# Borx25/CPU-Raytracing-experiments

Measured on AMD Instinct MI355X. Metric: Mray/s (primary+bounce), higher is better.
Workload: dtype f32; 1 GPU; cfg4: 4096x4096 px, S(100000) spheres + SAH BVH, MIS, Policy.max_bounces=9 (primary+8 bounces), 5 buckets, 64 accumulations/step; fixed image, tile rows split over the GPUs; image=4096x4096, spheres=100000, max_bounces=9, buckets=5, parallelism=single GPU, batches_in_flight=1, accumulations_per_batch=63, accumulations_per_batch_limit=63

## Files before the change

cpu-raytracing-experiments_amd/csrc/kernels.hpp:

```cpp
#pragma once
#include <hip/hip_runtime.h>
#include <stdint.h>
#include "device_math.hpp"

namespace mirt {

constexpr uint32_t kBlock = 256;
constexpr uint32_t kShadeBlock = 512;
constexpr uint32_t kTraceBlock = 1024;
constexpr uint32_t kLdsStack = 16;
constexpr uint32_t kLdsStackWide = 12;
constexpr uint32_t kLeafBit = 0x80000000u;
constexpr uint32_t kTileSize = 256;
constexpr uint32_t kTileRoot = 16;
constexpr uint32_t kStack = 64;
constexpr uint32_t kDestAccum = 0x80000000u;

struct SceneDev {
	const float4* recs;
	const float4* spheres;
	const int32_t* prim_mat;
	const float4* light_sphere;
	const float4* light_emit;
	const float4* mat_albedo;
// ... 578 lines not shown
		out.path[i] = path;
	}
}

template <int MODE, bool COUNT, class LoadRay, class StoreResult>
MIRT_DI void trace_queue(const SceneDev& sc, const TraceLds tl, const Queue& q, uint32_t n, uint32_t* work_next, FatList fat, uint32_t& c_nodes, uint32_t& c_spheres,
                         LoadRay load_ray, StoreResult store_result, const Collect col = Collect{ nullptr, 0.0f, 0u }) {
	if (n == 0) return;
	const bool all = bvh_all_in_lds(sc);
	if (sc.half_boxes && sc.wide) {
		if (!sc.stack16) trace_persistent<MODE, COUNT, false, true, false, true>(sc, tl, q, n, work_next, fat, c_nodes, c_spheres, load_ray, store_result, col);
		else if (all) trace_persistent<MODE, COUNT, true, true, true, true>(sc, tl, q, n, work_next, fat, c_nodes, c_spheres, load_ray, store_result, col);
		else trace_persistent<MODE, COUNT, false, true, true, true>(sc, tl, q, n, work_next, fat, c_nodes, c_spheres, load_ray, store_result, col);
	} else if (sc.half_boxes) {
		if (!sc.stack16) trace_persistent<MODE, COUNT, false, true, false, false>(sc, tl, q, n, work_next, fat, c_nodes, c_spheres, load_ray, store_result, col);
		else if (all) trace_persistent<MODE, COUNT, true, true, true, false>(sc, tl, q, n, work_next, fat, c_nodes, c_spheres, load_ray, store_result, col);
		else trace_persistent<MODE, COUNT, false, true, true, false>(sc, tl, q, n, work_next, fat, c_nodes, c_spheres, load_ray, store_result, col);
	} else {
		if (all) trace_persistent<MODE, COUNT, true, false, false, false>(sc, tl, q, n, work_next, fat, c_nodes, c_spheres, load_ray, store_result, col);
		else trace_persistent<MODE, COUNT, false, false, false, false>(sc, tl, q, n, work_next, fat, c_nodes, c_spheres, load_ray, store_result, col);
	}
}

MIRT_DI size_t accum_index(uint32_t acc_base, uint32_t buckets, uint32_t pix_bits, uint32_t path) {
	const uint32_t slot = path >> pix_bits;
	const uint32_t pix = path & ((1u << pix_bits) - 1u);
	const uint32_t bucket = (acc_base + slot + 1u) % buckets;
	return (static_cast<size_t>(pix >> 8) * buckets + bucket) * 3u * kTileSize + (pix & 255u);
}
MIRT_DI size_t accum_index(const FrameParams& fp, uint32_t path) { return accum_index(fp.idx_base, fp.idx_buckets, fp.pix_bits, path); }
MIRT_DI void accumulate_add(float* __restrict__ accum, size_t idx, float r, float g, float b) {
	accum[idx] += r; accum[idx + kTileSize] += g; accum[idx + 2 * kTileSize] += b;
}
constexpr uint32_t kDestFull = 0x40000000u;
constexpr uint32_t kDestSlot = 0x3fffffffu;
struct ShadowSink {
	float *rr, *rg, *rb;
	const float *px, *py, *pz;
	float* accum;
	uint32_t acc_base, buckets, pix_bits;
	uint32_t* occ;
};
MIRT_DI void shadow_origin(const ShadowBuf& sh, const ShadowSink& sink, uint32_t i, float& px, float& py, float& pz) {
	if (sink.occ) { px = sh.px[i]; py = sh.py[i]; pz = sh.pz[i]; return; }
	const uint32_t dw = sh.dest[i];
	if (dw & kDestAccum) { px = sh.px[i]; py = sh.py[i]; pz = sh.pz[i]; }
	else { const uint32_t d = dw & kDestSlot; px = sink.px[d]; py = sink.py[d]; pz = sink.pz[d]; }
}
MIRT_DI void shadow_finish(const ShadowBuf& sh, const ShadowSink& sink, uint32_t i, bool occluded, uint32_t& c_term) {
	if (sink.occ) { sink.occ[i] = occluded ? 1u : 0u; return; }
	const uint32_t dw = sh.dest[i];
	const uint32_t dest = dw & (kDestSlot | kDestAccum);
	if (dw & kDestAccum) c_term++;
	if (dw & kDestFull) {
		f3 R{ sh.rr[i], sh.rg[i], sh.rb[i] };
		const f3 E{ sh.er[i], sh.eg[i], sh.eb[i] };
		if (!occluded) { R.x += sh.sr[i]; R.y += sh.sg[i]; R.z += sh.sb[i]; }
		R.x += E.x; R.y += E.y; R.z += E.z;
		if (dest & kDestAccum) accumulate_add(sink.accum, accum_index(sink.acc_base, sink.buckets, sink.pix_bits, dest & ~kDestAccum), R.x, R.y, R.z);
		else { sink.rr[dest] = R.x; sink.rg[dest] = R.y; sink.rb[dest] = R.z; }
	} else if (!occluded) {
		const f3 S{ sh.sr[i], sh.sg[i], sh.sb[i] };
		if (dest & kDestAccum) accumulate_add(sink.accum, accum_index(sink.acc_base, sink.buckets, sink.pix_bits, dest & ~kDestAccum), S.x, S.y, S.z);
		else { sink.rr[dest] += S.x; sink.rg[dest] += S.y; sink.rb[dest] += S.z; }
	}
}

constexpr int kPrimaryNone = 0, kPrimaryAll = 1, kPrimaryList = 2;
MIRT_DI uint32_t primary_list_ray(const FrameParams& fp, const uint32_t* __restrict__ ov_pix, uint32_t n_ov, float inv_n_ov, uint32_t j) {
	uint32_t k;
	const uint32_t slot = udiv_f(j, n_ov, inv_n_ov, k);
	return slot * fp.n_pix + ov_pix[k];
}
template <bool COUNT, int PRIMARY>
__global__ __launch_bounds__(kTraceBlock, 8) void k_trace(SceneDev sc, FrameParams fp,
                                                       StreamBuf in, HitRec* __restrict__ hit_out,
                                                       Queue closest_queue, uint32_t* closest_work,
                                                       ShadowBuf sh, ShadowSink sink,
                                                       Queue shadow_queue, uint32_t* shadow_work, FatList fat_closest, FatList fat_shadow,
                                                       DevCounters* ctr) {
	extern __shared__ float4 lds[];
	const uint32_t n_ov = PRIMARY == kPrimaryList ? closest_queue.n[0] : 0u;
	const float inv_n_ov = 1.0f / static_cast<float>(n_ov ? n_ov : 1u);
	if (PRIMARY) closest_queue.n = nullptr;
	const uint32_t nc = PRIMARY == kPrimaryAll ? fp.n_pix * fp.batch_n : PRIMARY == kPrimaryList ? n_ov * fp.batch_n : queue_total(closest_queue), ns = PRIMARY ? 0u : queue_total(shadow_queue);
	if (nc + ns == 0) return;
	if (blockIdx.x == 0 && threadIdx.x == 0) {
		if (nc && PRIMARY != kPrimaryList) atomicAdd(&ctr->rays, static_cast<unsigned long long>(nc));
		if (ns) atomicAdd(&ctr->shadow_rays, static_cast<unsigned long long>(ns));
	}
	uint32_t c_nodes = 0, c_spheres = 0, s_nodes = 0, s_spheres = 0, c_term = 0;
	if (sc.use_bvh && sc.n_recs != 0) {
		if (static_cast<uint64_t>(blockIdx.x) * 64u >= static_cast<uint64_t>(nc) + ns) return;
		const TraceLds tl = stage_bvh(sc, lds);
		{
			auto load_ray = [&](uint32_t i, float& px, float& py, float& pz, float& dx, float& dy, float& dz, float& tf) {
// ... 231 lines not shown
			}
			lane_on = pix < fp.n_pix;
			my_slot = slot_it * fp.n_pix + pix;
			if (lane_on) {
				uint32_t rng = hash_2d(fp.acc_base + slot_it + 1u, pix_seed);
				const float s0 = rand_unit_float(rng);
				const float s1 = rand_unit_float(rng);
				my_D = camera_ray_dir(fp.cam, pix_x, pix_y, s0, s1);
				my_path = (slot_it << fp.pix_bits) | pix;
				{ const HitRec h = hit_in[my_slot]; my_prim = h.prim; my_tfar = h.tfar; }
			}
			if (++slot_it == slot_end) unit += gridDim.x;
		} else {
			lane_on = base + threadIdx.x < n;
			const uint32_t nb = base + gridDim.x * kShadeBlock;
			next_slot = (nb + threadIdx.x < n) ? queue_slot(qin, nb, nb + threadIdx.x) : 0u;
			next_prim = hit_in[next_slot].prim;
			base = nb;
		}
		{
			if (lane_on) {
				const uint32_t i = my_slot;
				const int32_t prim = my_prim;
				if (prim < 0) {
					f3 R{0.0f, 0.0f, 0.0f};
					float thr_x = 1.0f;
					uint32_t mpath = my_path; f3 md = my_D;
					if (!FIRST) { R = { in.rr[i], in.rg[i], in.rb[i] }; thr_x = in.tr[i]; mpath = in.path[i]; }
					if (sc.has_ambient) {
						if (!FIRST) md = { in.dx[i], in.dy[i], in.dz[i] };
						const f3 sky = sky_eval(sc, md.x, md.y, md.z);
						R.x += thr_x * sky.x; R.y += thr_x * sky.y; R.z += thr_x * sky.z;
					}
					accumulate_add(accum, accum_index(fp, mpath), R.x + 0.0f, R.y + 0.0f, R.z + 0.0f);
					c_term++;
				} else if (last_bounce) {
					c_drop++;
				} else is_hit = true;
			}
		}
		const uint32_t n_hits = FIRST ? 0u : block_compact(is_hit, my_slot, compact_scratch, hit_list);

		bool survive = false, has_shadow = false, terminated = false, has_E = false;
		uint32_t path = 0;
		f3 P{0, 0, 0}, ndir{0, 0, 0}, L{0, 0, 0}, srad{0, 0, 0}, E{0, 0, 0};
		f3 R{0.0f, 0.0f, 0.0f}, thr{1.0f, 1.0f, 1.0f};
		float light_distance = 0.0f;
		if (FIRST ? is_hit : threadIdx.x < n_hits) {
			const uint32_t i = FIRST ? my_slot : hit_list[threadIdx.x];
			f3 D = my_D;
			path = my_path;
			if (!FIRST) { path = in.path[i]; D = { in.dx[i], in.dy[i], in.dz[i] }; }
			float pdf_in = 0.0f;
			if (!FIRST) {
				R = { in.rr[i], in.rg[i], in.rb[i] };
				thr = { in.tr[i], in.tg[i], in.tb[i] };
				pdf_in = MIRT_INV_PI * max_sel(0.0f, D.z);
			}
			const HitRec hrec = FIRST ? HitRec{ my_tfar, my_prim } : hit_in[i];
			const int32_t prim = hrec.prim;
			{
				const float depth = hrec.tfar;
				const float4 hs = sc.spheres[prim];
				const int32_t mat = sc.prim_mat[prim];
				const f3 O = FIRST ? f3{ fp.cam.pos[0], fp.cam.pos[1], fp.cam.pos[2] } : f3{ in.px[i], in.py[i], in.pz[i] };
				const f3 hit{ O.x + D.x * depth, O.y + D.y * depth, O.z + D.z * depth };
				f3 N = normalize3(f3{ hit.x - hs.x, hit.y - hs.y, hit.z - hs.z });
				if (dot3(N, D) >= 0.0f) N = f3{ -N.x, -N.y, -N.z };
				const quat T = tangent_space(N);
				const f3 Vl = to_local(T, f3{ -D.x, -D.y, -D.z });
// ... 42 lines not shown
					} while (false);
				}
				has_E = is_emissive;
				if (is_emissive) {
					if (fp.mis && bounce > 0) {
						const float radius2 = hs.w;
						const float center_dist2 = depth * (depth + Vl.z * (2.0f * __builtin_sqrtf(radius2))) + radius2;
						const float weight = powerHeuristic(pdf_in, light_selection_pdf * spherePdf(radius2, center_dist2));
						E = { (thr.x * weight) * em.x, (thr.y * weight) * em.y, (thr.z * weight) * em.z };
					} else {
						E = { em.x, em.y, em.z };
					}
				}
				{
					uint32_t rng = hash_2d(acc, seed + bounce * 2u + 1u);
					const float b0 = rand_unit_float(rng);
					const float b1 = rand_unit_float(rng);
					f3 sd = hemisphere(b0, b1);
					thr = { thr.x * alb.x, thr.y * alb.y, thr.z * alb.z };
					const float q = 1.0f - max_sel(thr.x, max_sel(thr.y, thr.z));
					if (rand_unit_float(rng) < q) {
						terminated = true;
					} else {
						const float inv = 1.0f / max_sel(MIRT_FLT_EPSILON, 1.0f - q);
						thr = { thr.x * inv, thr.y * inv, thr.z * inv };
						ndir = to_world(T, sd);
						survive = true;
					}
				}
			}
		}
		uint32_t slot, sslot;
		block_append2(survive, has_shadow, next_queue, shadow_queue, iteration % kSegs, append_scratch, parity, slot, sslot);
		const bool direct = fp.idx_base != 0xffffffffu;
		const bool full = has_shadow & (has_E | (terminated & direct));
		if (survive) {
			out.px[slot] = P.x; out.py[slot] = P.y; out.pz[slot] = P.z;
			out.dx[slot] = ndir.x; out.dy[slot] = ndir.y; out.dz[slot] = ndir.z;
			out.tr[slot] = thr.x; out.tg[slot] = thr.y; out.tb[slot] = thr.z;
			out.path[slot] = path;
		}
		if (has_shadow) {
			if (!survive) { sh.px[sslot] = P.x; sh.py[sslot] = P.y; sh.pz[sslot] = P.z; }
			sh.dx[sslot] = L.x; sh.dy[sslot] = L.y; sh.dz[sslot] = L.z;
			sh.tfar[sslot] = light_distance;
			sh.sr[sslot] = srad.x; sh.sg[sslot] = srad.y; sh.sb[sslot] = srad.z;
			if (full) {
				sh.rr[sslot] = R.x; sh.rg[sslot] = R.y; sh.rb[sslot] = R.z;
				sh.er[sslot] = E.x; sh.eg[sslot] = E.y; sh.eb[sslot] = E.z;
			}
			sh.dest[sslot] = (survive ? slot : (kDestAccum | path)) | (full ? kDestFull : 0u);
		}
		if ((survive | terminated) & !full) {
			const f3 Rf{ R.x + E.x, R.y + E.y, R.z + E.z };
			if (survive) { out.rr[slot] = Rf.x; out.rg[slot] = Rf.y; out.rb[slot] = Rf.z; }
			else accumulate_add(accum, accum_index(fp, path), Rf.x, Rf.y, Rf.z);
		}
		c_term += (terminated && !has_shadow) ? 1u : 0u;
	}
	wave_sum(c_term, &ctr->terminated);
	wave_sum(c_drop, &ctr->dropped);
}

__global__ __launch_bounds__(kBlock) void k_merge_contrib(float4* __restrict__ accum, const float4* __restrict__ contrib, uint32_t n_tiles, uint32_t buckets,
                                                          uint32_t batch_n, uint32_t acc_base) {
	constexpr uint32_t kQuads = 3u * kTileSize / 4u;
	const size_t n_items = static_cast<size_t>(n_tiles) * kQuads;
	const uint32_t first = min(buckets, batch_n);
	for (size_t item = static_cast<size_t>(blockIdx.x) * kBlock + threadIdx.x; item < n_items; item += static_cast<size_t>(gridDim.x) * kBlock) {
		const size_t tile = item / kQuads; const uint32_t q = static_cast<uint32_t>(item % kQuads);
		for (uint32_t k0 = 0; k0 < first; k0++) {
			const uint32_t bucket = (acc_base + k0 + 1u) % buckets;
			float4* dst = accum + (tile * buckets + bucket) * kQuads + q;
			float4 a = *dst;
			for (uint32_t k = k0; k < batch_n; k += buckets) {
				const float4 c = contrib[(tile * batch_n + k) * kQuads + q];
				a.x += c.x; a.y += c.y; a.z += c.z; a.w += c.w;
			}
			*dst = a;
		}
	}
}

MIRT_DI float median_k(float* v, uint32_t k) {
	if (k == 5) return median5(v[0], v[1], v[2], v[3], v[4]);
	for (uint32_t a = 1; a < k; a++) {
		float key = v[a]; int b = static_cast<int>(a) - 1;
		while (b >= 0 && key < v[b]) { v[b + 1] = v[b]; b--; }
		v[b + 1] = key;
	}
	return (k & 1u) ? v[k / 2] : (v[k / 2 - 1] + v[k / 2]) * 0.5f;
}
__global__ __launch_bounds__(kBlock) void k_resolve(const float* __restrict__ accum, float4* __restrict__ fb, uint32_t n_pix, uint32_t first_tile,
                                                    uint32_t run_tiles, uint32_t stride_tiles, uint32_t h_tiles, uint32_t width, uint32_t buckets, float scale) {
	for (uint32_t pix = blockIdx.x * kBlock + threadIdx.x; pix < n_pix; pix += gridDim.x * kBlock) {
		const float* src = accum + static_cast<size_t>(pix >> 8) * buckets * 3u * kTileSize + (pix & 255u);
		float ch[3];
		for (uint32_t c = 0; c < 3; c++) {
			float v[16];
			for (uint32_t b = 0; b < 16; b++) if (b < buckets) v[b] = src[(static_cast<size_t>(b) * 3u + c) * kTileSize];
			ch[c] = scale * median_k(v, buckets);
		}
		tonemapping(ch[0], ch[1], ch[2]);
		const uint32_t tile = global_tile(first_tile, run_tiles, stride_tiles, pix >> 8), ID = pix & 255u;
		const uint32_t x = kTileRoot * (tile % h_tiles) + (ID & 15u);
		const uint32_t y = kTileRoot * (tile / h_tiles) + (ID >> 4);
		fb[static_cast<size_t>(y) * width + x] = make_float4(ch[0], ch[1], ch[2], 1.0f);
	}
}

__global__ __launch_bounds__(kBlock) void k_debug_math(int fn, uint32_t n, const float* in, float* out) {
	for (uint32_t i = blockIdx.x * kBlock + threadIdx.x; i < n; i += gridDim.x * kBlock) {
// ... 44 lines not shown
```

cpu-raytracing-experiments_amd/csrc/mirt_capi.hip:

```cpp
#include "../../include/mirt.h"
#include "kernels.hpp"
#include "bvh_layout.hpp"
#include "bvh_build.hpp"
#include "lbvh_build.hpp"

#include <hip/hip_runtime.h>
#include <algorithm>
#include <cstdarg>
#include <cstdio>
#include <cstdlib>
#include <cstring>
#include <string>
#include <vector>

using namespace mirt;

namespace {

thread_local std::string g_create_error;

struct DeviceBuffer {
	void* ptr = nullptr;
	size_t bytes = 0;
	hipError_t ensure(size_t want) {
		if (want <= bytes && ptr) return hipSuccess;
		if (ptr) { (void)hipFree(ptr); ptr = nullptr; bytes = 0; }
		if (want == 0) return hipSuccess;
		hipError_t e = hipMalloc(&ptr, want);
		if (e == hipSuccess) bytes = want;
		return e;
	}
	void release() { if (ptr) (void)hipFree(ptr); ptr = nullptr; bytes = 0; }
	template <class T> T* as() const { return static_cast<T*>(ptr); }
};

struct ScopedBuffer : DeviceBuffer {
	ScopedBuffer() = default;
	ScopedBuffer(const ScopedBuffer&) = delete;
	ScopedBuffer& operator=(const ScopedBuffer&) = delete;
	~ScopedBuffer() { release(); }
};

struct TimedLaunch { int klass; hipEvent_t start, stop; };

struct PipeSlot {
	hipStream_t stream = nullptr;
	DeviceBuffer arena;
	DeviceBuffer counts;
	DeviceBuffer contrib;
	DeviceBuffer fat;
	DeviceBuffer cand;
	hipEvent_t batch_done = nullptr;
	hipEvent_t merged = nullptr;
	hipEvent_t zeroed = nullptr;
	bool contrib_is_zero = false;
	bool zero_pending = false;
	bool in_use = false;
	StreamBuf stream_buf[2]{};
	ShadowBuf shadow_buf{};
	HitRec* hit = nullptr;
};

}

struct mirt_ctx {
	int device = 0;
	int n_cu = 256;
	hipStream_t stream = nullptr;
	hipStream_t side_stream = nullptr;
	std::string error;

	mirt_policy policy{ 16, 5, 1, 0, 0, 0, 0, 0, 0, 0, 0, { 0 } };
	uint32_t width = 0, height = 0, h_tiles = 0, v_tiles = 0;
	uint32_t first_tile = 0, n_tiles = 0;
	uint32_t run_tiles = 0, stride_tiles = 0;
	uint32_t accumulations = 0;
	bool have_scene = false, have_camera = false;

	DeviceBuffer recs, recs_wide, spheres, prim_mat, light_sphere, light_emit, mat_albedo, mat_emission, hdri;
	SceneDev scene{};
	CameraParams camera{};
	uint32_t trace_lds_bytes = 0;
	uint32_t bvh_depth = 0;
	bool allow_half = true;

	DeviceBuffer accumulator;
	DeviceBuffer framebuffer;
	float* frame_host = nullptr;
	size_t frame_host_bytes = 0;
	DeviceBuffer counters;
	std::vector<PipeSlot> slots;
	uint64_t planned_for = 0;
	uint32_t batch_mem_cap = 256;
	uint32_t capacity = 0;
	uint32_t seg_cap = 0;
	uint32_t arena_bounces = 0;
	uint64_t batch_seq = 0;

	uint32_t deferred = 0;
	uint32_t tune_trace_wgs = 2, tune_shade_wgs = 3, tune_chunk = kChunkMax, tune_leaf_batch = kLeafBatch, tune_refill_idle = kRefillIdle, tune_wide = 1, tune_zero_ahead = 1;
	std::vector<TimedLaunch> pending;
	std::vector<hipEvent_t> free_events;
	mirt_kernel_times times{};
};

namespace {

int fail(mirt_ctx* ctx, int code, const char* fmt, ...) {
	char buf[512];
	va_list ap; va_start(ap, fmt); vsnprintf(buf, sizeof buf, fmt, ap); va_end(ap);
	if (ctx) ctx->error = buf; else g_create_error = buf;
	return code;
}
#define HIP_TRY(ctx, expr) do { hipError_t _e = (expr); if (_e != hipSuccess) return fail(ctx, MIRT_ERR_HIP, "%s: %s", #expr, hipGetErrorString(_e)); } while (0)

constexpr uint32_t kMaxBatch = 256;
constexpr uint64_t kBatchRays = 1024ull << 20;
constexpr uint64_t kSerialRays = 96ull << 20;
constexpr size_t kStreamPlanes = 2 * 13 + 2 + 17;
uint32_t pix_bits_of(const mirt_ctx* c) { uint32_t b = 8; while ((1ull << b) < static_cast<uint64_t>(c->n_tiles) * kTileSize) b++; return b; }
uint32_t max_slots(const mirt_ctx* c) {
	const uint64_t n_pix = std::max<uint64_t>(static_cast<uint64_t>(c->n_tiles) * kTileSize, 1);
	const uint64_t by_slots = ((1ull << 30) - 3ull * kSegs * kShadeBlock) / n_pix;
	return static_cast<uint32_t>(std::max<uint64_t>(std::min<uint64_t>(std::min<uint64_t>(kMaxBatch, 1u << (30u - std::min<uint32_t>(pix_bits_of(c), 24u))), by_slots), 1));
}
uint32_t batch_floor(const mirt_ctx* c) { return std::max<uint32_t>(std::min<uint32_t>(c->policy.buckets, 5u), 1u); }
uint32_t batch_limit(const mirt_ctx* c) {
	if (c->policy.max_batch) return std::min(c->policy.max_batch, max_slots(c));
	const uint64_t n_pix = static_cast<uint64_t>(c->n_tiles) * kTileSize;
	if (n_pix == 0) return 1;
	const uint64_t b = std::max<uint64_t>((kBatchRays + n_pix / 2) / n_pix, batch_floor(c));
	return static_cast<uint32_t>(std::min<uint64_t>(std::min<uint64_t>(b, max_slots(c)), std::max<uint32_t>(c->batch_mem_cap, 1u)));
}
bool uses_contrib(const mirt_ctx* c, uint32_t n_slots) { return n_slots > 1 || batch_limit(c) > c->policy.buckets; }

uint32_t grid_for(const mirt_ctx* c, uint64_t work_items) {
	uint64_t blocks = (work_items + kBlock - 1) / kBlock;
	const uint64_t cap = static_cast<uint64_t>(c->n_cu) * 8u;
	if (blocks > cap) blocks = cap;
	if (blocks < 1) blocks = 1;
	return static_cast<uint32_t>(blocks);
}

constexpr uint32_t kLdsPerCu = 160u * 1024u;
uint32_t stack_bytes(bool half, bool stack16) { return half ? (stack16 ? kLdsStack * kTraceBlock * 2u : kLdsStackWide * kTraceBlock * 4u) : kLdsStack * kTraceBlock * 4u; }
uint32_t stack_bytes(const mirt_ctx* c) { return stack_bytes(c->scene.half_boxes != 0, c->scene.stack16 != 0); }
uint32_t stage_budget(bool half, bool stack16) { return half ? (stack16 ? 48u * 1024u : 32u * 1024u) : 96u * 1024u; }
uint32_t trace_lds(const mirt_ctx* c) { return c->policy.use_bvh ? c->trace_lds_bytes + stack_bytes(c) : kBruteChunk * 16u; }
uint32_t trace_grid(const mirt_ctx* c, uint64_t work_items) {
	uint32_t per_cu = kLdsPerCu / trace_lds(c);
	if (per_cu > c->tune_trace_wgs) per_cu = c->tune_trace_wgs;
	if (per_cu < 1) per_cu = 1;
	uint64_t blocks = (work_items + kTraceBlock - 1) / kTraceBlock;
	const uint64_t cap = static_cast<uint64_t>(c->n_cu) * per_cu;
	if (blocks > cap) blocks = cap;
	if (blocks < 1) blocks = 1;
	return static_cast<uint32_t>(blocks);
}

hipError_t sync_all(mirt_ctx* c) {
	for (PipeSlot& sl : c->slots) if (sl.stream) { hipError_t e = hipStreamSynchronize(sl.stream); if (e != hipSuccess) return e; }
	if (c->side_stream) { hipError_t e = hipStreamSynchronize(c->side_stream); if (e != hipSuccess) return e; }
	return hipStreamSynchronize(c->stream);
}
constexpr uint32_t kQueueWords = kSegs * kSegPitch;
size_t counts_words(uint32_t nb) { return static_cast<size_t>(2 * nb + 2) * kQueueWords + static_cast<size_t>(nb) * 4 + 8; }
constexpr uint32_t kFatCapacity = 1u << 16;
uint32_t wanted_slots(const mirt_ctx* c) {
	if (c->policy.streams) return std::min<uint32_t>(c->policy.streams, 8u);
	return static_cast<uint64_t>(c->n_tiles) * kTileSize * batch_limit(c) >= kSerialRays ? 1u : 3u;
}
uint64_t streams_bytes(const mirt_ctx* c) {
	const uint64_t rays = static_cast<uint64_t>(c->n_tiles) * kTileSize * batch_limit(c);
	return wanted_slots(c) * (rays * 4u * kStreamPlanes + (uses_contrib(c, wanted_slots(c)) ? rays * 12u : 0u));
}

void plan_batches(mirt_ctx* c) {
	const uint64_t n_pix = static_cast<uint64_t>(c->n_tiles) * kTileSize;
	if (c->policy.max_batch || n_pix == 0 || c->planned_for == n_pix) return;
	c->batch_mem_cap = kMaxBatch;
	size_t free_b = 0, total_b = 0, own = 0;
	for (const PipeSlot& sl : c->slots) own += sl.arena.bytes + sl.contrib.bytes;
	if (hipSetDevice(c->device) == hipSuccess && hipMemGetInfo(&free_b, &total_b) == hipSuccess)
		while (batch_limit(c) > batch_floor(c) && streams_bytes(c) > (free_b + own) / 5 * 4) c->batch_mem_cap = std::max(batch_limit(c) / 2, batch_floor(c));
	c->planned_for = n_pix;
}

int ensure_streams(mirt_ctx* c) {
	const uint64_t n_pix = static_cast<uint64_t>(c->n_tiles) * kTileSize;
	if (n_pix * batch_limit(c) == 0) return MIRT_OK;
	plan_batches(c);
	const uint64_t cap64 = n_pix * batch_limit(c);
	if (n_pix > (1u << 24)) return fail(c, MIRT_ERR_ARG, "more than 2^24 pixels per context (%llu); shard the tile range", (unsigned long long)n_pix);
	if (cap64 + 3ull * kSegs * kShadeBlock > (1ull << 30)) return fail(c, MIRT_ERR_ARG, "stream capacity %llu too large", (unsigned long long)cap64);
	const uint32_t seg_cap = static_cast<uint32_t>((((cap64 + kShadeBlock - 1) / kShadeBlock + kSegs - 1) / kSegs + 2) * kShadeBlock);
	const uint32_t cap = seg_cap * kSegs;
	const uint32_t nb = c->policy.max_bounces;
	const uint32_t want = wanted_slots(c);
	const bool contrib = uses_contrib(c, want);
	const size_t acc_bytes = static_cast<size_t>(c->n_tiles) * batch_limit(c) * 3 * kTileSize * sizeof(float);
	if (cap == c->capacity && nb == c->arena_bounces && c->slots.size() == want && (!contrib || c->slots[0].contrib.bytes >= acc_bytes)) return MIRT_OK;
	HIP_TRY(c, sync_all(c));
	while (c->slots.size() > want) {
		PipeSlot& sl = c->slots.back();
		sl.arena.release(); sl.counts.release(); sl.contrib.release(); sl.fat.release(); sl.cand.release();
		if (sl.batch_done) (void)hipEventDestroy(sl.batch_done);
		if (sl.merged) (void)hipEventDestroy(sl.merged);
		if (sl.zeroed) (void)hipEventDestroy(sl.zeroed);
		if (sl.stream) (void)hipStreamDestroy(sl.stream);
		c->slots.pop_back();
	}
	while (c->slots.size() < want) {
		PipeSlot sl;
		HIP_TRY(c, hipStreamCreateWithFlags(&sl.stream, hipStreamNonBlocking));
		HIP_TRY(c, hipEventCreateWithFlags(&sl.batch_done, hipEventDisableTiming));
		HIP_TRY(c, hipEventCreateWithFlags(&sl.merged, hipEventDisableTiming));
		HIP_TRY(c, hipEventCreateWithFlags(&sl.zeroed, hipEventDisableTiming));
		c->slots.push_back(sl);
	}
	const size_t planes = kStreamPlanes;
	const size_t plane_bytes = (static_cast<size_t>(cap) * 4 + 255) & ~static_cast<size_t>(255);
	for (PipeSlot& sl : c->slots) {
		sl.in_use = false; sl.contrib_is_zero = false; sl.zero_pending = false;
		hipError_t e = sl.arena.ensure(planes * plane_bytes);
		const char* what = "ray streams";
		if (e == hipSuccess) { e = sl.counts.ensure(counts_words(nb) * sizeof(uint32_t)); what = "queue counters"; }
		if (e == hipSuccess) { e = sl.fat.ensure(2u * kFatCapacity * sizeof(uint32_t)); what = "fat-ray lists"; }
		if (e == hipSuccess) { e = sl.cand.ensure(static_cast<size_t>(n_pix) * kCandStride * sizeof(uint32_t)); what = "candidate lists"; }
		if (e == hipSuccess) { if (contrib) { e = sl.contrib.ensure(acc_bytes); what = "contribution buffer"; } else sl.contrib.release(); }
		if (e != hipSuccess) {
			(void)hipGetLastError();
			if (e == hipErrorOutOfMemory && !c->policy.max_batch && batch_limit(c) > batch_floor(c)) {
				for (PipeSlot& other : c->slots) { other.arena.release(); other.contrib.release(); }
				c->capacity = 0;
				c->batch_mem_cap = std::max(batch_limit(c) / 2, batch_floor(c));
				return ensure_streams(c);
			}
			return fail(c, MIRT_ERR_HIP, "%s (%zu bytes of ray streams per batch in flight): %s", what, planes * plane_bytes, hipGetErrorString(e));
		}
		char* p = sl.arena.as<char>();
		auto take = [&]() { void* r = p; p += plane_bytes; return r; };
		for (int b = 0; b < 2; b++) {
			StreamBuf& s = sl.stream_buf[b];
			s.px = (float*)take(); s.py = (float*)take(); s.pz = (float*)take();
			s.dx = (float*)take(); s.dy = (float*)take(); s.dz = (float*)take();
			s.tr = (float*)take(); s.tg = (float*)take(); s.tb = (float*)take();
			s.rr = (float*)take(); s.rg = (float*)take(); s.rb = (float*)take();
			s.path = (uint32_t*)take();
		}
		sl.hit = (HitRec*)take(); (void)take();
		ShadowBuf& h = sl.shadow_buf;
		h.px = (float*)take(); h.py = (float*)take(); h.pz = (float*)take();
		h.dx = (float*)take(); h.dy = (float*)take(); h.dz = (float*)take(); h.tfar = (float*)take();
		h.sr = (float*)take(); h.sg = (float*)take(); h.sb = (float*)take();
		h.rr = (float*)take(); h.rg = (float*)take(); h.rb = (float*)take();
		h.er = (float*)take(); h.eg = (float*)take(); h.eb = (float*)take();
// ... 48 lines not shown
FrameParams frame_params(const mirt_ctx* c, uint32_t acc_base, uint32_t batch_n) {
	FrameParams fp{};
	fp.cam = c->camera;
	fp.h_tiles = c->h_tiles;
	fp.first_tile = c->first_tile;
	fp.run_tiles = c->run_tiles ? c->run_tiles : 1u;
	fp.stride_tiles = c->stride_tiles;
	fp.n_pix = c->n_tiles * kTileSize;
	fp.pix_bits = pix_bits_of(c); fp.pix_mask = (1u << fp.pix_bits) - 1u;
	fp.acc_base = acc_base;
	fp.batch_n = batch_n;
	fp.idx_base = acc_base;
	fp.idx_buckets = c->policy.buckets;
	fp.max_bounces = c->policy.max_bounces;
	fp.buckets = c->policy.buckets;
	fp.n_lights = c->scene.n_lights;
	fp.mis = (c->policy.mis && c->scene.n_lights > 0) ? 1u : 0u;
	fp.first_groups = 1;
	fp.inv_n_pix = fp.n_pix ? 1.0f / static_cast<float>(fp.n_pix) : 0.0f;
	fp.inv_h_tiles = fp.h_tiles ? 1.0f / static_cast<float>(fp.h_tiles) : 0.0f;
	fp.inv_run_tiles = 1.0f / static_cast<float>(fp.run_tiles);
	return fp;
}

int launch_batch(mirt_ctx* c, uint32_t batch_n) {
	FrameParams fp = frame_params(c, c->accumulations, batch_n);
	const uint32_t nb = c->policy.max_bounces;
	const uint64_t total = static_cast<uint64_t>(fp.n_pix) * batch_n;
	if (total == 0) { c->accumulations += batch_n; return MIRT_OK; }
	const bool pipelined = c->slots.size() > 1;
	PipeSlot& sl = c->slots[c->batch_seq % c->slots.size()];
	hipStream_t st = pipelined ? sl.stream : c->stream;
	const bool contrib = uses_contrib(c, static_cast<uint32_t>(c->slots.size()));
	const size_t contrib_floats = static_cast<size_t>(c->n_tiles) * batch_n * 3 * kTileSize;
	if (contrib) { fp.idx_base = 0xffffffffu; fp.idx_buckets = batch_n; }
	uint32_t* counts = sl.counts.as<uint32_t>();
	auto stream_queue = [&](uint32_t b) { return Queue{ counts + static_cast<size_t>(b) * kQueueWords, c->seg_cap }; };
	auto shadow_queue = [&](uint32_t b) { return Queue{ counts + static_cast<size_t>(nb + 1 + b) * kQueueWords, c->seg_cap }; };
	const Queue empty_queue{ counts + static_cast<size_t>(2 * nb + 1) * kQueueWords, c->seg_cap };
	uint32_t* work_next = counts + static_cast<size_t>(2 * nb + 2) * kQueueWords;
	uint32_t* work_next_shadow = work_next + nb;
	uint32_t* fat_n_closest = work_next_shadow + nb;
	uint32_t* fat_n_shadow = fat_n_closest + nb;
	uint32_t* misc = fat_n_shadow + nb;
	const float qn = c->camera.orient[0] * c->camera.orient[0] + c->camera.orient[1] * c->camera.orient[1] + c->camera.orient[2] * c->camera.orient[2] + c->camera.orient[3] * c->camera.orient[3];
	const bool bundle = c->policy.use_bvh && c->scene.n_recs != 0 && !c->policy.trace_primary_rays && batch_n >= 3 && c->camera.z != 0.0f && std::fabs(qn - 1.0f) < 1e-4f;
	const float rho = bundle ? bundle_half_angle(c) : 0.0f;
	DevCounters* ctr = c->counters.as<DevCounters>();
	float* accum = contrib ? sl.contrib.as<float>() : c->accumulator.as<float>();
	SceneDev sc = c->scene;
	sc.use_bvh = c->policy.use_bvh;
	sc.chunk_max = c->tune_chunk; sc.leaf_batch = c->tune_leaf_batch; sc.refill_idle = c->tune_refill_idle;
	const bool count = c->policy.count_traffic != 0;
	const uint32_t tgrid = trace_grid(c, total);
	const uint32_t sgrid = static_cast<uint32_t>(std::min<uint64_t>((total + kShadeBlock - 1) / kShadeBlock, static_cast<uint64_t>(c->n_cu) * c->tune_shade_wgs));
	const uint32_t tlds = trace_lds(c);
	{
		const uint64_t n_chunks = (static_cast<uint64_t>(fp.n_pix) + kShadeBlock - 1) / kShadeBlock;
		const uint64_t want = (8ull * sgrid + n_chunks - 1) / n_chunks;
		fp.first_groups = static_cast<uint32_t>(std::min<uint64_t>(std::max<uint64_t>(want, 1), batch_n));
	}
	const uint32_t fat_grid = sc.n_spheres > 4096 ? static_cast<uint32_t>(c->n_cu) * 2u : 64u;

	if (pipelined && sl.in_use) HIP_TRY(c, hipStreamWaitEvent(st, sl.merged, 0));
	const bool zero_ahead = contrib && !pipelined && c->tune_zero_ahead;
	if (contrib && !(zero_ahead && sl.contrib_is_zero)) {
		HIP_TRY(c, hipMemsetAsync(sl.contrib.ptr, 0, zero_ahead ? sl.contrib.bytes : contrib_floats * sizeof(float), st));
		sl.contrib_is_zero = zero_ahead; sl.zero_pending = false;
	}
	HIP_TRY(c, hipMemsetAsync(counts, 0, counts_words(nb) * sizeof(uint32_t), st));
	for (uint32_t bounce = 0; bounce < nb; bounce++) {
		const StreamBuf& in = sl.stream_buf[bounce & 1u];
		const StreamBuf& out = sl.stream_buf[(bounce & 1u) ^ 1u];
		const bool shadow_pending = fp.mis && bounce > 0;
		{ Bracket t(c, MIRT_K_TRACE, st);
		  const Queue sq = shadow_pending ? shadow_queue(bounce - 1) : empty_queue;
		  uint32_t* sc_work = work_next_shadow + (shadow_pending ? bounce - 1 : 0);
		  const FatList fc{ fat_n_closest + bounce, sl.fat.as<uint32_t>(), kFatCapacity };
		  const FatList fs{ fat_n_shadow + bounce, sl.fat.as<uint32_t>() + kFatCapacity, kFatCapacity };
		  const ShadowSink sink{ in.rr, in.rg, in.rb, in.px, in.py, in.pz, accum, fp.idx_base, fp.idx_buckets, fp.pix_bits, nullptr };
		  const Queue cq = (bounce == 0 && bundle) ? Queue{ misc + 2, 0u } : stream_queue(bounce);
		  auto launch_trace = [&](auto kernel, auto fat_kernel) {
		    hipLaunchKernelGGL(kernel, dim3(tgrid), dim3(kTraceBlock), tlds, st, sc, fp, in, sl.hit, cq, work_next + bounce,
		                       sl.shadow_buf, sink, sq, sc_work, fc, fs, ctr);
		    if (sc.use_bvh) hipLaunchKernelGGL(fat_kernel, dim3(fat_grid), dim3(1024), 0, st, sc, fp, in, sl.hit, fc, sl.shadow_buf, sink, fs, ctr, misc + 2);
		  };
		  if (bounce == 0 && bundle) {
		    const FatList none{ misc + 1, sl.fat.as<uint32_t>(), 0u };
		    if (count) hipLaunchKernelGGL(k_primary_cand<true>, dim3(trace_grid(c, fp.n_pix)), dim3(kTraceBlock), tlds, st, sc, fp, sl.cand.as<uint32_t>(), rho, misc, none, ctr, in.path, misc + 2);
		    else       hipLaunchKernelGGL(k_primary_cand<false>, dim3(trace_grid(c, fp.n_pix)), dim3(kTraceBlock), tlds, st, sc, fp, sl.cand.as<uint32_t>(), rho, misc, none, ctr, in.path, misc + 2);
		    const uint32_t hgrid = static_cast<uint32_t>(std::min<uint64_t>((static_cast<uint64_t>(fp.n_pix) + kBlock - 1) / kBlock, static_cast<uint64_t>(c->n_cu) * 64u));
		    if (count) hipLaunchKernelGGL(k_primary_hits<true>, dim3(hgrid), dim3(kBlock), 0, st, sc, fp, sl.cand.as<uint32_t>(), sl.hit, ctr);
		    else       hipLaunchKernelGGL(k_primary_hits<false>, dim3(hgrid), dim3(kBlock), 0, st, sc, fp, sl.cand.as<uint32_t>(), sl.hit, ctr);
		    if (count) launch_trace((k_trace<true, kPrimaryList>), (k_trace_fat<true, kPrimaryList>)); else launch_trace((k_trace<false, kPrimaryList>), (k_trace_fat<false, kPrimaryList>));
		  }
		  else if (bounce == 0) { if (count) launch_trace((k_trace<true, kPrimaryAll>), (k_trace_fat<true, kPrimaryAll>)); else launch_trace((k_trace<false, kPrimaryAll>), (k_trace_fat<false, kPrimaryAll>)); }
		  else                  { if (count) launch_trace((k_trace<true, kPrimaryNone>), (k_trace_fat<true, kPrimaryNone>)); else launch_trace((k_trace<false, kPrimaryNone>), (k_trace_fat<false, kPrimaryNone>)); } }
		if (bounce == 0 && zero_ahead && sl.zero_pending) { HIP_TRY(c, hipStreamWaitEvent(st, sl.zeroed, 0)); sl.zero_pending = false; }
		{ Bracket t(c, MIRT_K_SHADE, st);
		  if (bounce == 0) hipLaunchKernelGGL(k_shade<true>, dim3(sgrid), dim3(kShadeBlock), 0, st, sc, fp, in, sl.hit, out, sl.shadow_buf, bounce, stream_queue(bounce), stream_queue(bounce + 1), shadow_queue(bounce), accum, ctr);
		  else             hipLaunchKernelGGL(k_shade<false>, dim3(sgrid), dim3(kShadeBlock), 0, st, sc, fp, in, sl.hit, out, sl.shadow_buf, bounce, stream_queue(bounce), stream_queue(bounce + 1), shadow_queue(bounce), accum, ctr); }
	}
	HIP_TRY(c, hipGetLastError());
	if (contrib) {
		if (pipelined) {
			HIP_TRY(c, hipEventRecord(sl.batch_done, st));
			HIP_TRY(c, hipStreamWaitEvent(c->stream, sl.batch_done, 0));
		}
		{ Bracket t(c, MIRT_K_RESOLVE);
		  hipLaunchKernelGGL(k_merge_contrib, dim3(grid_for(c, static_cast<uint64_t>(c->n_tiles) * (3u * kTileSize / 4u))), dim3(kBlock), 0, c->stream,
		                     c->accumulator.as<float4>(), sl.contrib.as<float4>(), c->n_tiles, c->policy.buckets, batch_n, fp.acc_base); }
		HIP_TRY(c, hipGetLastError());
		if (pipelined) { HIP_TRY(c, hipEventRecord(sl.merged, c->stream)); sl.in_use = true; }
		if (zero_ahead) {
			HIP_TRY(c, hipEventRecord(sl.merged, c->stream));
			HIP_TRY(c, hipStreamWaitEvent(c->side_stream, sl.merged, 0));
			HIP_TRY(c, hipMemsetAsync(sl.contrib.ptr, 0, contrib_floats * sizeof(float), c->side_stream));
			HIP_TRY(c, hipEventRecord(sl.zeroed, c->side_stream));
			sl.zero_pending = true;
		}
	}
	c->batch_seq++;
	c->accumulations += batch_n;
	if (c->policy.profile && c->pending.size() > 512) harvest(c);
	return MIRT_OK;
}

template <class T>
int upload(mirt_ctx* c, DeviceBuffer& buf, const std::vector<T>& host) {
	HIP_TRY(c, buf.ensure(std::max<size_t>(host.size(), 1) * sizeof(T)));
	if (!host.empty()) HIP_TRY(c, hipMemcpyAsync(buf.ptr, host.data(), host.size() * sizeof(T), hipMemcpyHostToDevice, c->stream));
	return MIRT_OK;
}

int check_ready(mirt_ctx* c) {
	if (!c) return MIRT_ERR_ARG;
	if (!c->have_scene) return fail(c, MIRT_ERR_STATE, "mirt_set_scene has not been called");
	if (!c->have_camera) return fail(c, MIRT_ERR_STATE, "mirt_set_camera has not been called");
	if (c->width == 0 && c->height == 0) return fail(c, MIRT_ERR_STATE, "mirt_resize has not been called");
	return MIRT_OK;
}

int flush_deferred(mirt_ctx* c) {
	if (!c->deferred) return MIRT_OK;
	const uint32_t n = c->deferred;
	c->deferred = 0;
	HIP_TRY(c, hipSetDevice(c->device));
	int r = ensure_streams(c); if (r) return r;
	return launch_batch(c, n);
}

}

extern "C" {

const char* mirt_last_error(const mirt_ctx* ctx) { return ctx ? ctx->error.c_str() : g_create_error.c_str(); }

int mirt_create(int device, mirt_ctx** out) {
	if (!out) return fail(nullptr, MIRT_ERR_ARG, "out is NULL");
	*out = nullptr;
	int n = 0;
	hipError_t e = hipGetDeviceCount(&n);
	if (e != hipSuccess || n <= 0) return fail(nullptr, MIRT_ERR_NO_DEVICE, "no HIP device available (%s); mirt has no CPU path", hipGetErrorString(e));
	if (device < 0 || device >= n) return fail(nullptr, MIRT_ERR_ARG, "device %d out of range (have %d)", device, n);
	e = hipSetDevice(device);
	if (e != hipSuccess) return fail(nullptr, MIRT_ERR_HIP, "hipSetDevice: %s", hipGetErrorString(e));
	mirt_ctx* c = new mirt_ctx();
	c->device = device;
	if (const char* e = std::getenv("MIRT_TUNE_CHUNK")) c->tune_chunk = static_cast<uint32_t>(std::min(std::max(std::atoi(e), 64), 65536)) & ~63u;
	if (const char* e = std::getenv("MIRT_TUNE_REFILL_IDLE")) c->tune_refill_idle = static_cast<uint32_t>(std::min(std::max(std::atoi(e), 1), 64));
	if (const char* e = std::getenv("MIRT_TUNE_ZERO_AHEAD")) c->tune_zero_ahead = std::atoi(e) != 0 ? 1u : 0u;
	if (const char* e = std::getenv("MIRT_TUNE_WIDE")) c->tune_wide = std::atoi(e) != 0 ? 1u : 0u;
	if (const char* e = std::getenv("MIRT_TUNE_LEAF_BATCH")) c->tune_leaf_batch = static_cast<uint32_t>(std::min(std::max(std::atoi(e), 1), 64));
	if (const char* e = std::getenv("MIRT_TUNE_TRACE_WGS")) c->tune_trace_wgs = std::atoi(e) == 1 ? 1u : 2u;
	if (const char* e = std::getenv("MIRT_TUNE_SHADE_WGS")) c->tune_shade_wgs = static_cast<uint32_t>(std::min(std::max(std::atoi(e), 1), 16));
	hipDeviceProp_t prop;
	if (hipGetDeviceProperties(&prop, device) == hipSuccess) c->n_cu = prop.multiProcessorCount > 0 ? prop.multiProcessorCount : 256;
	e = hipStreamCreateWithFlags(&c->stream, hipStreamNonBlocking);
	if (e == hipSuccess) e = hipStreamCreateWithFlags(&c->side_stream, hipStreamNonBlocking);
	if (e == hipSuccess) e = c->counters.ensure(sizeof(DevCounters));
	if (e == hipSuccess) e = hipMemsetAsync(c->counters.ptr, 0, sizeof(DevCounters), c->stream);
	if (e != hipSuccess) { int r = fail(nullptr, MIRT_ERR_HIP, "context setup: %s", hipGetErrorString(e)); delete c; return r; }
	*out = c;
	return MIRT_OK;
}

int mirt_destroy(mirt_ctx* c) {
	if (!c) return MIRT_ERR_ARG;
	(void)hipSetDevice(c->device);
	(void)sync_all(c);
	harvest(c);
	for (PipeSlot& sl : c->slots) {
		sl.arena.release(); sl.counts.release(); sl.contrib.release(); sl.fat.release(); sl.cand.release();
		if (sl.batch_done) (void)hipEventDestroy(sl.batch_done);
		if (sl.merged) (void)hipEventDestroy(sl.merged);
		if (sl.zeroed) (void)hipEventDestroy(sl.zeroed);
		if (sl.stream) (void)hipStreamDestroy(sl.stream);
	}
	c->slots.clear();
	for (hipEvent_t e : c->free_events) (void)hipEventDestroy(e);
	DeviceBuffer* bufs[] = { &c->recs, &c->recs_wide, &c->spheres, &c->prim_mat, &c->light_sphere, &c->light_emit, &c->mat_albedo, &c->mat_emission,
	                         &c->hdri, &c->accumulator, &c->framebuffer, &c->counters };
	for (DeviceBuffer* b : bufs) b->release();
	if (c->frame_host) (void)hipHostFree(c->frame_host);
	if (c->side_stream) (void)hipStreamDestroy(c->side_stream);
	if (c->stream) (void)hipStreamDestroy(c->stream);
	delete c;
	return MIRT_OK;
}

int mirt_set_scene(mirt_ctx* c, const mirt_sphere* geometry, const mirt_sphere* bvh_prims, uint32_t n_spheres,
                   const mirt_bvh_node* nodes, uint32_t n_nodes, const mirt_material* materials, uint32_t n_materials,
                   const int32_t* lights, uint32_t n_lights, const float ambient_color[3],
                   const float* hdri_rgba, uint32_t hdri_w, uint32_t hdri_h) {
	if (!c) return MIRT_ERR_ARG;
	{ const int fr = flush_deferred(c); if (fr) return fr; }
	if (n_spheres && (!geometry || !bvh_prims)) return fail(c, MIRT_ERR_ARG, "geometry / bvh_prims is NULL");
	if (n_spheres >= (1u << 26)) return fail(c, MIRT_ERR_ARG, "more than 2^26 spheres");
	if (n_nodes && !nodes) return fail(c, MIRT_ERR_ARG, "nodes is NULL");
	if (!materials || n_materials == 0 || n_materials > MIRT_MAX_MATERIALS) return fail(c, MIRT_ERR_ARG, "need 1..%u materials, got %u", MIRT_MAX_MATERIALS, n_materials);
	if (n_lights && !lights) return fail(c, MIRT_ERR_ARG, "lights is NULL");
	if (!ambient_color || !hdri_rgba || hdri_w == 0 || hdri_h == 0) return fail(c, MIRT_ERR_ARG, "sky needs ambient_color and an hdri of at least 1x1");
	for (uint32_t i = 0; i < n_spheres; i++) {
		if (geometry[i].material_ID < 0 || static_cast<uint32_t>(geometry[i].material_ID) >= n_materials ||
		    bvh_prims[i].material_ID < 0 || static_cast<uint32_t>(bvh_prims[i].material_ID) >= n_materials)
			return fail(c, MIRT_ERR_ARG, "sphere %u: material_ID out of range", i);
		for (const mirt_sphere* s : { &geometry[i], &bvh_prims[i] })
			if (!std::isfinite(s->position[0]) || !std::isfinite(s->position[1]) || !std::isfinite(s->position[2]) || !std::isfinite(s->radius_sq) || s->radius_sq < 0.0f)
				return fail(c, MIRT_ERR_ARG, "sphere %u: position / radius_sq must be finite, radius_sq >= 0", i);
	}
	for (uint32_t i = 0; i < n_lights; i++)
		if (lights[i] < 0 || static_cast<uint32_t>(lights[i]) >= n_spheres) return fail(c, MIRT_ERR_ARG, "light %u: index out of range", i);
	{
		std::vector<uint8_t> has_parent(n_nodes, 0);
		for (uint32_t i = 0; i < n_nodes; i++) {
			const mirt_bvh_node& nd = nodes[i];
			if (nd.prim_count == 0) {
				if (nd.first_id <= i || static_cast<uint64_t>(nd.first_id) + 1 >= n_nodes) return fail(c, MIRT_ERR_ARG, "node %u: child index %u invalid", i, nd.first_id);
// ... 458 lines not shown
```

Baseline: 8437 Mray/s.

## Write path contributions directly instead of zero-filling the contrib buffer

New measurement: 8986 Mray/s, median of 6. 6.5% higher.

```diff
diff --git a/cpu-raytracing-experiments_amd/csrc/kernels.hpp b/cpu-raytracing-experiments_amd/csrc/kernels.hpp
--- a/cpu-raytracing-experiments_amd/csrc/kernels.hpp
+++ b/cpu-raytracing-experiments_amd/csrc/kernels.hpp
@@ -634,6 +634,25 @@
 MIRT_DI void accumulate_add(float* __restrict__ accum, size_t idx, float r, float g, float b) {
 	accum[idx] += r; accum[idx + kTileSize] += g; accum[idx + 2 * kTileSize] += b;
 }
+constexpr uint32_t kIdxContrib = 0xffffffffu;
+MIRT_DI size_t contrib_index(uint32_t batch_n, uint32_t pix_bits, uint32_t path) {
+	const uint32_t slot = path >> pix_bits;
+	const uint32_t pix = path & ((1u << pix_bits) - 1u);
+	return ((static_cast<size_t>(pix >> 8) * batch_n + slot) * kTileSize + (pix & 255u)) * 3u;
+}
+MIRT_DI void path_result(float* __restrict__ accum, uint32_t idx_base, uint32_t idx_buckets, uint32_t pix_bits, uint32_t path, float r, float g, float b) {
+	if (idx_base == kIdxContrib) {
+		float* w = accum + contrib_index(idx_buckets, pix_bits, path);
+		w[0] = 0.0f + r; w[1] = 0.0f + g; w[2] = 0.0f + b;
+	} else accumulate_add(accum, accum_index(idx_base, idx_buckets, pix_bits, path), r, g, b);
+}
+MIRT_DI void path_result_add(float* __restrict__ accum, uint32_t idx_base, uint32_t idx_buckets, uint32_t pix_bits, uint32_t path, float r, float g, float b) {
+	if (idx_base == kIdxContrib) {
+		float* w = accum + contrib_index(idx_buckets, pix_bits, path);
+		w[0] += r; w[1] += g; w[2] += b;
+	} else accumulate_add(accum, accum_index(idx_base, idx_buckets, pix_bits, path), r, g, b);
+}
+MIRT_DI void path_result(float* __restrict__ accum, const FrameParams& fp, uint32_t path, float r, float g, float b) { path_result(accum, fp.idx_base, fp.idx_buckets, fp.pix_bits, path, r, g, b); }
 constexpr uint32_t kDestFull = 0x40000000u;
 constexpr uint32_t kDestSlot = 0x3fffffffu;
 struct ShadowSink {
@@ -659,11 +678,11 @@
 		const f3 E{ sh.er[i], sh.eg[i], sh.eb[i] };
 		if (!occluded) { R.x += sh.sr[i]; R.y += sh.sg[i]; R.z += sh.sb[i]; }
 		R.x += E.x; R.y += E.y; R.z += E.z;
-		if (dest & kDestAccum) accumulate_add(sink.accum, accum_index(sink.acc_base, sink.buckets, sink.pix_bits, dest & ~kDestAccum), R.x, R.y, R.z);
+		if (dest & kDestAccum) path_result(sink.accum, sink.acc_base, sink.buckets, sink.pix_bits, dest & ~kDestAccum, R.x, R.y, R.z);
 		else { sink.rr[dest] = R.x; sink.rg[dest] = R.y; sink.rb[dest] = R.z; }
 	} else if (!occluded) {
 		const f3 S{ sh.sr[i], sh.sg[i], sh.sb[i] };
-		if (dest & kDestAccum) accumulate_add(sink.accum, accum_index(sink.acc_base, sink.buckets, sink.pix_bits, dest & ~kDestAccum), S.x, S.y, S.z);
+		if (dest & kDestAccum) path_result_add(sink.accum, sink.acc_base, sink.buckets, sink.pix_bits, dest & ~kDestAccum, S.x, S.y, S.z);
 		else { sink.rr[dest] += S.x; sink.rg[dest] += S.y; sink.rb[dest] += S.z; }
 	}
 }
@@ -961,10 +980,14 @@
 						const f3 sky = sky_eval(sc, md.x, md.y, md.z);
 						R.x += thr_x * sky.x; R.y += thr_x * sky.y; R.z += thr_x * sky.z;
 					}
-					accumulate_add(accum, accum_index(fp, mpath), R.x + 0.0f, R.y + 0.0f, R.z + 0.0f);
+					path_result(accum, fp, mpath, R.x + 0.0f, R.y + 0.0f, R.z + 0.0f);
 					c_term++;
 				} else if (last_bounce) {
 					c_drop++;
+					if (fp.idx_base == kIdxContrib) {
+						float* w = accum + contrib_index(fp.idx_buckets, fp.pix_bits, FIRST ? my_path : in.path[i]);
+						w[0] = 0.0f; w[1] = 0.0f; w[2] = 0.0f;
+					}
 				} else is_hit = true;
 			}
 		}
@@ -1073,7 +1096,7 @@
 		}
 		uint32_t slot, sslot;
 		block_append2(survive, has_shadow, next_queue, shadow_queue, iteration % kSegs, append_scratch, parity, slot, sslot);
-		const bool direct = fp.idx_base != 0xffffffffu;
+		const bool direct = fp.idx_base != kIdxContrib;
 		const bool full = has_shadow & (has_E | (terminated & direct));
 		if (survive) {
 			out.px[slot] = P.x; out.py[slot] = P.y; out.pz[slot] = P.z;
@@ -1095,7 +1118,7 @@
 		if ((survive | terminated) & !full) {
 			const f3 Rf{ R.x + E.x, R.y + E.y, R.z + E.z };
 			if (survive) { out.rr[slot] = Rf.x; out.rg[slot] = Rf.y; out.rb[slot] = Rf.z; }
-			else accumulate_add(accum, accum_index(fp, path), Rf.x, Rf.y, Rf.z);
+			else path_result(accum, fp, path, Rf.x, Rf.y, Rf.z);
 		}
 		c_term += (terminated && !has_shadow) ? 1u : 0u;
 	}
@@ -1105,20 +1128,24 @@
 
 __global__ __launch_bounds__(kBlock) void k_merge_contrib(float4* __restrict__ accum, const float4* __restrict__ contrib, uint32_t n_tiles, uint32_t buckets,
                                                           uint32_t batch_n, uint32_t acc_base) {
-	constexpr uint32_t kQuads = 3u * kTileSize / 4u;
+	constexpr uint32_t kQuads = kTileSize / 4u;
 	const size_t n_items = static_cast<size_t>(n_tiles) * kQuads;
 	const uint32_t first = min(buckets, batch_n);
 	for (size_t item = static_cast<size_t>(blockIdx.x) * kBlock + threadIdx.x; item < n_items; item += static_cast<size_t>(gridDim.x) * kBlock) {
 		const size_t tile = item / kQuads; const uint32_t q = static_cast<uint32_t>(item % kQuads);
 		for (uint32_t k0 = 0; k0 < first; k0++) {
 			const uint32_t bucket = (acc_base + k0 + 1u) % buckets;
-			float4* dst = accum + (tile * buckets + bucket) * kQuads + q;
-			float4 a = *dst;
+			float4* dst = accum + (tile * buckets + bucket) * 3u * kQuads + q;
+			float4 r = dst[0], g = dst[kQuads], b = dst[2u * kQuads];
 			for (uint32_t k = k0; k < batch_n; k += buckets) {
-				const float4 c = contrib[(tile * batch_n + k) * kQuads + q];
-				a.x += c.x; a.y += c.y; a.z += c.z; a.w += c.w;
+				const float4* src = contrib + ((tile * batch_n + k) * kQuads + q) * 3u;
+				const float4 c0 = src[0], c1 = src[1], c2 = src[2];
+				r.x += c0.x; g.x += c0.y; b.x += c0.z;
+				r.y += c0.w; g.y += c1.x; b.y += c1.y;
+				r.z += c1.z; g.z += c1.w; b.z += c2.x;
+				r.w += c2.y; g.w += c2.z; b.w += c2.w;
 			}
-			*dst = a;
+			dst[0] = r; dst[kQuads] = g; dst[2u * kQuads] = b;
 		}
 	}
 }
diff --git a/cpu-raytracing-experiments_amd/csrc/mirt_capi.hip b/cpu-raytracing-experiments_amd/csrc/mirt_capi.hip
--- a/cpu-raytracing-experiments_amd/csrc/mirt_capi.hip
+++ b/cpu-raytracing-experiments_amd/csrc/mirt_capi.hip
@@ -52,9 +52,6 @@
 	DeviceBuffer cand;
 	hipEvent_t batch_done = nullptr;
 	hipEvent_t merged = nullptr;
-	hipEvent_t zeroed = nullptr;
-	bool contrib_is_zero = false;
-	bool zero_pending = false;
 	bool in_use = false;
 	StreamBuf stream_buf[2]{};
 	ShadowBuf shadow_buf{};
@@ -67,7 +64,6 @@
 	int device = 0;
 	int n_cu = 256;
 	hipStream_t stream = nullptr;
-	hipStream_t side_stream = nullptr;
 	std::string error;
 
 	mirt_policy policy{ 16, 5, 1, 0, 0, 0, 0, 0, 0, 0, 0, { 0 } };
@@ -98,7 +94,8 @@
 	uint64_t batch_seq = 0;
 
 	uint32_t deferred = 0;
-	uint32_t tune_trace_wgs = 2, tune_shade_wgs = 3, tune_chunk = kChunkMax, tune_leaf_batch = kLeafBatch, tune_refill_idle = kRefillIdle, tune_wide = 1, tune_zero_ahead = 1;
+	uint32_t tune_trace_wgs = 2, tune_shade_wgs = 3, tune_chunk = kChunkMax, tune_leaf_batch = kLeafBatch, tune_refill_idle = kRefillIdle, tune_wide = 1;
+	bool debug_poison_contrib = false;
 	std::vector<TimedLaunch> pending;
 	std::vector<hipEvent_t> free_events;
 	mirt_kernel_times times{};
@@ -160,7 +157,6 @@
 
 hipError_t sync_all(mirt_ctx* c) {
 	for (PipeSlot& sl : c->slots) if (sl.stream) { hipError_t e = hipStreamSynchronize(sl.stream); if (e != hipSuccess) return e; }
-	if (c->side_stream) { hipError_t e = hipStreamSynchronize(c->side_stream); if (e != hipSuccess) return e; }
 	return hipStreamSynchronize(c->stream);
 }
 constexpr uint32_t kQueueWords = kSegs * kSegPitch;
@@ -206,7 +202,6 @@
 		sl.arena.release(); sl.counts.release(); sl.contrib.release(); sl.fat.release(); sl.cand.release();
 		if (sl.batch_done) (void)hipEventDestroy(sl.batch_done);
 		if (sl.merged) (void)hipEventDestroy(sl.merged);
-		if (sl.zeroed) (void)hipEventDestroy(sl.zeroed);
 		if (sl.stream) (void)hipStreamDestroy(sl.stream);
 		c->slots.pop_back();
 	}
@@ -215,13 +210,12 @@
 		HIP_TRY(c, hipStreamCreateWithFlags(&sl.stream, hipStreamNonBlocking));
 		HIP_TRY(c, hipEventCreateWithFlags(&sl.batch_done, hipEventDisableTiming));
 		HIP_TRY(c, hipEventCreateWithFlags(&sl.merged, hipEventDisableTiming));
-		HIP_TRY(c, hipEventCreateWithFlags(&sl.zeroed, hipEventDisableTiming));
 		c->slots.push_back(sl);
 	}
 	const size_t planes = kStreamPlanes;
 	const size_t plane_bytes = (static_cast<size_t>(cap) * 4 + 255) & ~static_cast<size_t>(255);
 	for (PipeSlot& sl : c->slots) {
-		sl.in_use = false; sl.contrib_is_zero = false; sl.zero_pending = false;
+		sl.in_use = false;
 		hipError_t e = sl.arena.ensure(planes * plane_bytes);
 		const char* what = "ray streams";
 		if (e == hipSuccess) { e = sl.counts.ensure(counts_words(nb) * sizeof(uint32_t)); what = "queue counters"; }
@@ -336,8 +330,7 @@
 	PipeSlot& sl = c->slots[c->batch_seq % c->slots.size()];
 	hipStream_t st = pipelined ? sl.stream : c->stream;
 	const bool contrib = uses_contrib(c, static_cast<uint32_t>(c->slots.size()));
-	const size_t contrib_floats = static_cast<size_t>(c->n_tiles) * batch_n * 3 * kTileSize;
-	if (contrib) { fp.idx_base = 0xffffffffu; fp.idx_buckets = batch_n; }
+	if (contrib) { fp.idx_base = kIdxContrib; fp.idx_buckets = batch_n; }
 	uint32_t* counts = sl.counts.as<uint32_t>();
 	auto stream_queue = [&](uint32_t b) { return Queue{ counts + static_cast<size_t>(b) * kQueueWords, c->seg_cap }; };
 	auto shadow_queue = [&](uint32_t b) { return Queue{ counts + static_cast<size_t>(nb + 1 + b) * kQueueWords, c->seg_cap }; };
@@ -367,11 +360,8 @@
 	const uint32_t fat_grid = sc.n_spheres > 4096 ? static_cast<uint32_t>(c->n_cu) * 2u : 64u;
 
 	if (pipelined && sl.in_use) HIP_TRY(c, hipStreamWaitEvent(st, sl.merged, 0));
-	const bool zero_ahead = contrib && !pipelined && c->tune_zero_ahead;
-	if (contrib && !(zero_ahead && sl.contrib_is_zero)) {
-		HIP_TRY(c, hipMemsetAsync(sl.contrib.ptr, 0, zero_ahead ? sl.contrib.bytes : contrib_floats * sizeof(float), st));
-		sl.contrib_is_zero = zero_ahead; sl.zero_pending = false;
-	}
+	if (contrib && c->debug_poison_contrib)
+		HIP_TRY(c, hipMemsetD32Async(reinterpret_cast<hipDeviceptr_t>(sl.contrib.ptr), 0x7fc0deadu, sl.contrib.bytes / sizeof(float), st));
 	HIP_TRY(c, hipMemsetAsync(counts, 0, counts_words(nb) * sizeof(uint32_t), st));
 	for (uint32_t bounce = 0; bounce < nb; bounce++) {
 		const StreamBuf& in = sl.stream_buf[bounce & 1u];
@@ -400,7 +390,6 @@
 		  }
 		  else if (bounce == 0) { if (count) launch_trace((k_trace<true, kPrimaryAll>), (k_trace_fat<true, kPrimaryAll>)); else launch_trace((k_trace<false, kPrimaryAll>), (k_trace_fat<false, kPrimaryAll>)); }
 		  else                  { if (count) launch_trace((k_trace<true, kPrimaryNone>), (k_trace_fat<true, kPrimaryNone>)); else launch_trace((k_trace<false, kPrimaryNone>), (k_trace_fat<false, kPrimaryNone>)); } }
-		if (bounce == 0 && zero_ahead && sl.zero_pending) { HIP_TRY(c, hipStreamWaitEvent(st, sl.zeroed, 0)); sl.zero_pending = false; }
 		{ Bracket t(c, MIRT_K_SHADE, st);
 		  if (bounce == 0) hipLaunchKernelGGL(k_shade<true>, dim3(sgrid), dim3(kShadeBlock), 0, st, sc, fp, in, sl.hit, out, sl.shadow_buf, bounce, stream_queue(bounce), stream_queue(bounce + 1), shadow_queue(bounce), accum, ctr);
 		  else             hipLaunchKernelGGL(k_shade<false>, dim3(sgrid), dim3(kShadeBlock), 0, st, sc, fp, in, sl.hit, out, sl.shadow_buf, bounce, stream_queue(bounce), stream_queue(bounce + 1), shadow_queue(bounce), accum, ctr); }
@@ -412,17 +401,10 @@
 			HIP_TRY(c, hipStreamWaitEvent(c->stream, sl.batch_done, 0));
 		}
 		{ Bracket t(c, MIRT_K_RESOLVE);
-		  hipLaunchKernelGGL(k_merge_contrib, dim3(grid_for(c, static_cast<uint64_t>(c->n_tiles) * (3u * kTileSize / 4u))), dim3(kBlock), 0, c->stream,
+		  hipLaunchKernelGGL(k_merge_contrib, dim3(grid_for(c, static_cast<uint64_t>(c->n_tiles) * (kTileSize / 4u))), dim3(kBlock), 0, c->stream,
 		                     c->accumulator.as<float4>(), sl.contrib.as<float4>(), c->n_tiles, c->policy.buckets, batch_n, fp.acc_base); }
 		HIP_TRY(c, hipGetLastError());
 		if (pipelined) { HIP_TRY(c, hipEventRecord(sl.merged, c->stream)); sl.in_use = true; }
-		if (zero_ahead) {
-			HIP_TRY(c, hipEventRecord(sl.merged, c->stream));
-			HIP_TRY(c, hipStreamWaitEvent(c->side_stream, sl.merged, 0));
-			HIP_TRY(c, hipMemsetAsync(sl.contrib.ptr, 0, contrib_floats * sizeof(float), c->side_stream));
-			HIP_TRY(c, hipEventRecord(sl.zeroed, c->side_stream));
-			sl.zero_pending = true;
-		}
 	}
 	c->batch_seq++;
 	c->accumulations += batch_n;
@@ -473,15 +455,14 @@
 	c->device = device;
 	if (const char* e = std::getenv("MIRT_TUNE_CHUNK")) c->tune_chunk = static_cast<uint32_t>(std::min(std::max(std::atoi(e), 64), 65536)) & ~63u;
 	if (const char* e = std::getenv("MIRT_TUNE_REFILL_IDLE")) c->tune_refill_idle = static_cast<uint32_t>(std::min(std::max(std::atoi(e), 1), 64));
-	if (const char* e = std::getenv("MIRT_TUNE_ZERO_AHEAD")) c->tune_zero_ahead = std::atoi(e) != 0 ? 1u : 0u;
 	if (const char* e = std::getenv("MIRT_TUNE_WIDE")) c->tune_wide = std::atoi(e) != 0 ? 1u : 0u;
 	if (const char* e = std::getenv("MIRT_TUNE_LEAF_BATCH")) c->tune_leaf_batch = static_cast<uint32_t>(std::min(std::max(std::atoi(e), 1), 64));
 	if (const char* e = std::getenv("MIRT_TUNE_TRACE_WGS")) c->tune_trace_wgs = std::atoi(e) == 1 ? 1u : 2u;
 	if (const char* e = std::getenv("MIRT_TUNE_SHADE_WGS")) c->tune_shade_wgs = static_cast<uint32_t>(std::min(std::max(std::atoi(e), 1), 16));
+	if (const char* e = std::getenv("MIRT_DEBUG_POISON_CONTRIB")) c->debug_poison_contrib = std::atoi(e) != 0;
 	hipDeviceProp_t prop;
 	if (hipGetDeviceProperties(&prop, device) == hipSuccess) c->n_cu = prop.multiProcessorCount > 0 ? prop.multiProcessorCount : 256;
 	e = hipStreamCreateWithFlags(&c->stream, hipStreamNonBlocking);
-	if (e == hipSuccess) e = hipStreamCreateWithFlags(&c->side_stream, hipStreamNonBlocking);
 	if (e == hipSuccess) e = c->counters.ensure(sizeof(DevCounters));
 	if (e == hipSuccess) e = hipMemsetAsync(c->counters.ptr, 0, sizeof(DevCounters), c->stream);
 	if (e != hipSuccess) { int r = fail(nullptr, MIRT_ERR_HIP, "context setup: %s", hipGetErrorString(e)); delete c; return r; }
@@ -498,7 +479,6 @@
 		sl.arena.release(); sl.counts.release(); sl.contrib.release(); sl.fat.release(); sl.cand.release();
 		if (sl.batch_done) (void)hipEventDestroy(sl.batch_done);
 		if (sl.merged) (void)hipEventDestroy(sl.merged);
-		if (sl.zeroed) (void)hipEventDestroy(sl.zeroed);
 		if (sl.stream) (void)hipStreamDestroy(sl.stream);
 	}
 	c->slots.clear();
@@ -507,7 +487,6 @@
 	                         &c->hdri, &c->accumulator, &c->framebuffer, &c->counters };
 	for (DeviceBuffer* b : bufs) b->release();
 	if (c->frame_host) (void)hipHostFree(c->frame_host);
-	if (c->side_stream) (void)hipStreamDestroy(c->side_stream);
 	if (c->stream) (void)hipStreamDestroy(c->stream);
 	delete c;
 	return MIRT_OK;
```
